# jonathanventura/spherical-sfm

Measured on AMD Instinct MI355X. Metric: BA obs/sec (Jac+Schur+PCG), higher is better.
Workload: dtype f64; 1 GPU; 300 cams x 100000 pts x 600000 obs synthetic circle (BASELINE configs[1]), general BA, focal fixed, CauchyLoss(1.0), Ceres-default LM; camera_dof=6, comm=none, reduced_solver=band-cholesky (direct), pcg_sweeps=0

## Files before the change

### spherical_sfm_amd/csrc/ba_kernels.h

```cpp
#pragma once
#include <hip/hip_runtime.h>
#include "ssfm_math.h"
#include "det_acc.h"

namespace ssfm {

static __global__ void k_profile_pad() {}

enum {
    SC_COST = 0,
    SC_FJJ = 1,
    SC_FJR = 2,
    SC_FWW = 3,
    SC_FWG = 4,
    SC_MODEL = 5,
    SC_STEP2_PT = 6,
    SC_XN2_PT = 7,
    SC_CAND_COST = 8,
    SC_X0N2_PT = 9,
    SC_NSUM = 10,
    SC_GMAX = 10,
    SC_STEP2_CAM = 11, SC_XN2_CAM = 12, SC_X0N2_CAM = 13,
    SC_TOTAL = 16
};
// ... 570 lines not shown
struct OctTR<N, 0> { static __device__ __forceinline__ void run(double (&v)[N], double* out) {
#pragma unroll
    for (int j = 0; j < N; j++) out[j] = v[j]; } };
__device__ __forceinline__ void wave_lds_handover() {
    __builtin_amdgcn_fence(__ATOMIC_RELEASE, "wavefront"); __builtin_amdgcn_wave_barrier(); __builtin_amdgcn_fence(__ATOMIC_ACQUIRE, "wavefront");
}
template <int DC> __device__ __forceinline__ constexpr bool jc_zero(int r, int i) { return DC == 6 && ((r == 0 && i == 1) || (r == 1 && i == 0)); }
__device__ __forceinline__ int gram_cam_of(int camv, int k) { return __shfl(camv, k, 64); }
template <int PER, int STRIDE, int NA>
__device__ __forceinline__ void gram_gather(const double* __restrict__ A, const double* __restrict__ B, int camv, int K, int lane, double* __restrict__ dst) {
    constexpr int NIT = (GRAM_KMAX * PER + 63) / 64;
    double v[NIT];
#pragma unroll
    for (int it = 0; it < NIT; it++) {
        const int e = lane + 64 * it, k = e / PER, i = e - PER * k;
        const int c = gram_cam_of(camv, min(k, K - 1));
        const double* src = (i < NA) ? A + 6 * (size_t)c + i : B + 27 * (size_t)c + (i - NA);
        v[it] = *src;
    }
#pragma unroll
    for (int it = 0; it < NIT; it++) {
        const int e = lane + 64 * it, k = e / PER, i = e - PER * k;
        if (e < K * PER) dst[k * STRIDE + i] = v[it];
    }
}
struct GramFuse { const double* scale_pt; double radius, min_diag, max_diag; double* PS_out; double* gp_out; double* scal; const double* spec; int emit_skip = 0; };
template <int DC, int NT, int TI, bool FUSE>
__device__ __forceinline__ void
schur_gram_task(const double* __restrict__ cam, const double* __restrict__ rot, const double* __restrict__ pts, const double* __restrict__ focal,
                const double2* __restrict__ obs_xy, const int* __restrict__ gr_rec, const double* __restrict__ scale_cam, const double* __restrict__ scale_f,
                const double* __restrict__ PS, int loss, double la, int rows_alloc, int focal_free, const int task, double* __restrict__ S_val, double* __restrict__ rhs,
                double* __restrict__ Udiag, double* __restrict__ Sfc, double* __restrict__ gcraw, long long* __restrict__ dbg, const GramFuse& fz, const DetZone& dz) {
    double fz_radius = fz.radius;
    if (FUSE && fz.spec) { if (fz.spec[0] == 0.0) return; fz_radius = fz.spec[1]; }
    constexpr int BB = DC * DC, off = (DC == 6) ? 0 : 3;
    constexpr int NU = DC * (DC + 1) / 2, NS = NU + 3 * DC, NO = (NS + 7) / 8;
    typedef double v4d_ __attribute__((ext_vector_type(4)));
    const long long t_0 = dbg ? wall_clock64() : 0;
    extern __shared__ __attribute__((aligned(16))) double sY[];
    const int lane = threadIdx.x & 63;
    double* sYw = sY + (size_t)(threadIdx.x >> 6) * (rows_alloc * GRAM_LD + GRAM_TAIL);
    double* sCam = sYw + rows_alloc * GRAM_LD;
    double* sScale = sCam + GRAM_KMAX * GRAM_CAMREC;
    int* sSlot = (int*)(sScale + 48);
    int* sDiag = sSlot + GRAM_NPAIR;
    const int* rec = gr_rec + (size_t)task * GRAM_REC;
    const int p0 = __builtin_amdgcn_readfirstlane(rec[0]), cnt = __builtin_amdgcn_readfirstlane(rec[1]), K = __builtin_amdgcn_readfirstlane(rec[2]);
    const int j00 = __builtin_amdgcn_readfirstlane(rec[3]);
    const double f = focal[0];
    const int camv = rec[4 + (lane & (GRAM_KMAX - 1))];
    gram_gather<33, GRAM_CAMREC, 6>(cam, rot, camv, K, lane, sCam);
    { const int k = min(lane / DC, K - 1), c = gram_cam_of(camv, k); const double sc = scale_cam[6 * c + off + lane - DC * (lane / DC)]; if (lane < DC * K) sScale[lane] = sc; }
    if (lane < GRAM_NPAIR + GRAM_KMAX) sSlot[lane] = rec[12 + lane];
    v4d_ acc[NT * (NT + 1) / 2];
#pragma unroll
    for (int t = 0; t < NT * (NT + 1) / 2; t++) acc[t] = v4d_{0.0, 0.0, 0.0, 0.0};
    double tacc[TI > 0 ? TI : 1] = {};
    double sm[NS];
#pragma unroll
    for (int i = 0; i < NS; i++) sm[i] = 0.0;
    const int li = lane & 15, lk = lane >> 4;
    const int lp = lane & (GRAM_SUB - 1), lq = lane >> 3;
    const int kq = min(lq, K - 1);
    const double sf = scale_f[0];
    double X[3], V[12]; double2 ob;
    double spt[3] = {0.0, 0.0, 0.0};
    double pacc[5] = {0.0, 0.0, 0.0, 0.0, 0.0}, pgmax = 0.0;
#define GRAM_LOAD(s0_)                                                                                                            \
    do {                                                                                                                          \
        const int q_ = min((s0_) + lp, cnt - 1);                                                                                  \
        _Pragma("unroll") for (int k = 0; k < 3; k++) X[k] = pts[3 * (size_t)(p0 + q_) + k];                                      \
        if (FUSE) { _Pragma("unroll") for (int k = 0; k < 3; k++) spt[k] = fz.scale_pt[3 * (size_t)(p0 + q_) + k]; }              \
        else {                                                                                                                    \
        _Pragma("unroll") for (int k = 0; k < 9; k++) V[k] = PS[12 * (size_t)(p0 + q_) + k];                                      \
        if (focal_free) { _Pragma("unroll") for (int k = 9; k < 12; k++) V[k] = PS[12 * (size_t)(p0 + q_) + k]; }                 \
        }                                                                                                                         \
        ob = obs_xy[j00 + (size_t)q_ * K + kq];                                                                                   \
    } while (0)
    GRAM_LOAD(0);
    long long t_1 = 0, t_2 = 0;
    for (int s0 = 0; s0 < cnt; s0 += GRAM_SUB) {
        wave_lds_handover();
        {
            const bool valid = s0 + lp < cnt;
            const double* crec = sCam + kq * GRAM_CAMREC;
            if (FUSE) {
                const double wgt = (valid && lq < K) ? 1.0 : 0.0;
                double pv[12];
                {
                    ObsPoint Lp; lin_obs_point(f, crec, crec + 6, X, ob.x, ob.y, loss, la, Lp);
                    double j0[2], j1[2], j2[2], jf[2];
#pragma unroll
                    for (int a = 0; a < 2; a++) { j0[a] = Lp.Jp[a][0] * spt[0] * wgt; j1[a] = Lp.Jp[a][1] * spt[1] * wgt; j2[a] = Lp.Jp[a][2] * spt[2] * wgt; jf[a] = Lp.Jf[a] * sf * wgt; }
                    pv[0] = j0[0] * j0[0] + j0[1] * j0[1]; pv[1] = j0[0] * j1[0] + j0[1] * j1[1]; pv[2] = j0[0] * j2[0] + j0[1] * j2[1];
                    pv[3] = j1[0] * j1[0] + j1[1] * j1[1]; pv[4] = j1[0] * j2[0] + j1[1] * j2[1]; pv[5] = j2[0] * j2[0] + j2[1] * j2[1];
                    pv[6] = j0[0] * Lp.r[0] + j0[1] * Lp.r[1]; pv[7] = j1[0] * Lp.r[0] + j1[1] * Lp.r[1]; pv[8] = j2[0] * Lp.r[0] + j2[1] * Lp.r[1];
                    pv[9] = jf[0] * j0[0] + jf[1] * j0[1]; pv[10] = jf[0] * j1[0] + jf[1] * j1[1]; pv[11] = jf[0] * j2[0] + jf[1] * j2[1];
                    pacc[0] += wgt * Lp.half_rho; pacc[1] += jf[0] * jf[0] + jf[1] * jf[1]; pacc[2] += jf[0] * Lp.r[0] + jf[1] * Lp.r[1];
                }
#pragma unroll
                for (int i = 0; i < 12; i++) { double t = pv[i]; t += __shfl_xor(t, 8, 64); t += __shfl_xor(t, 16, 64); t += __shfl_xor(t, 32, 64); pv[i] = t; }
                double Vd[6] = {pv[0], pv[1], pv[2], pv[3], pv[4], pv[5]};
                if (spt[0] > 0.0) {
                    if (valid && lq == 0) pgmax = fmax(pgmax, fmax(fabs(pv[6] / spt[0]), fmax(fabs(pv[7] / spt[1]), fabs(pv[8] / spt[2]))));
                    Vd[0] += fmin(fmax(Vd[0], fz.min_diag), fz.max_diag) / fz_radius;
                    Vd[3] += fmin(fmax(Vd[3], fz.min_diag), fz.max_diag) / fz_radius;
                    Vd[5] += fmin(fmax(Vd[5], fz.min_diag), fz.max_diag) / fz_radius;
                } else { Vd[0] = Vd[3] = Vd[5] = 1.0; }
                double Vi[6]; sym3_inverse(Vd, Vi);
                const double u0 = pv[9] * Vi[0] + pv[10] * Vi[1] + pv[11] * Vi[2];
                const double u1 = pv[9] * Vi[1] + pv[10] * Vi[3] + pv[11] * Vi[4];
                const double u2 = pv[9] * Vi[2] + pv[10] * Vi[4] + pv[11] * Vi[5];
                V[0] = Vi[0] * spt[0] * spt[0]; V[1] = Vi[1] * spt[0] * spt[1]; V[2] = Vi[2] * spt[0] * spt[2];
                V[3] = Vi[3] * spt[1] * spt[1]; V[4] = Vi[4] * spt[1] * spt[2]; V[5] = Vi[5] * spt[2] * spt[2];
                V[6] = spt[0] * (Vi[0] * pv[6] + Vi[1] * pv[7] + Vi[2] * pv[8]); V[7] = spt[1] * (Vi[1] * pv[6] + Vi[3] * pv[7] + Vi[4] * pv[8]);
                V[8] = spt[2] * (Vi[2] * pv[6] + Vi[4] * pv[7] + Vi[5] * pv[8]);
                V[9] = spt[0] * u0; V[10] = spt[1] * u1; V[11] = spt[2] * u2;
                if (valid && lq == 0) {
                    pacc[3] += u0 * pv[9] + u1 * pv[10] + u2 * pv[11];
                    pacc[4] += u0 * pv[6] + u1 * pv[7] + u2 * pv[8];
                    double* ps = fz.PS_out + 12 * (size_t)(p0 + s0 + lp);
#pragma unroll
                    for (int k = 0; k < 12; k++) ps[k] = V[k];
#pragma unroll
                    for (int k = 0; k < 3; k++) fz.gp_out[3 * (size_t)(p0 + s0 + lp) + k] = pv[6 + k];
                }
            }
            ObsLin Lk; lin_obs<DC == 6>(f, crec, crec + 6, X, ob.x, ob.y, loss, la, Lk);
            double L00 = 0, L10 = 0, L20 = 0, L11 = 0, L21 = 0, L22 = 0;
            if (valid && V[0] > 0.0) {
                const double i0 = fast_rsqrt(V[0]);
                L00 = V[0] * i0; L10 = V[1] * i0; L20 = V[2] * i0;
                const double d1 = V[3] - L10 * L10;
                if (d1 > 0.0) {
                    const double i1 = fast_rsqrt(d1);
                    L11 = d1 * i1; L21 = (V[4] - L20 * L10) * i1;
                    const double d2 = V[5] - L20 * L20 - L21 * L21;
                    if (d2 > 0.0) L22 = d2 * fast_rsqrt(d2);
                }
            }
            double Jc[2][DC]; cam_block_raw<DC>(Lk, Jc);
            double T[2][3];
#pragma unroll
            for (int r = 0; r < 2; r++) {
                T[r][0] = Lk.Jp[r][0] * L00 + Lk.Jp[r][1] * L10 + Lk.Jp[r][2] * L20;
                T[r][1] = Lk.Jp[r][1] * L11 + Lk.Jp[r][2] * L21;
                T[r][2] = Lk.Jp[r][2] * L22;
            }
            if (lq < K) {
                double* dst = sYw + (size_t)(DC * kq) * GRAM_LD + 3 * lp;
#pragma unroll
                for (int d = 0; d < DC; d++)
#pragma unroll
                    for (int cc = 0; cc < 3; cc++) {
                        double y = 0.0;
                        if (!jc_zero<DC>(0, d)) y += Jc[0][d] * T[0][cc];
                        if (!jc_zero<DC>(1, d)) y += Jc[1][d] * T[1][cc];
                        dst[d * GRAM_LD + cc] = y;
                    }
                if (valid) {
                    double yv[2], zv[2];
#pragma unroll
                    for (int r = 0; r < 2; r++) {
                        yv[r] = Lk.Jp[r][0] * V[6] + Lk.Jp[r][1] * V[7] + Lk.Jp[r][2] * V[8];
                        zv[r] = focal_free ? Lk.Jf[r] * sf - (Lk.Jp[r][0] * V[9] + Lk.Jp[r][1] * V[10] + Lk.Jp[r][2] * V[11]) : 0.0;
                    }
                    int u = 0;
#pragma unroll
                    for (int a2 = 0; a2 < DC; a2++) {
#pragma unroll
                        for (int b2 = a2; b2 < DC; b2++) {
                            if (!jc_zero<DC>(0, a2) && !jc_zero<DC>(0, b2)) sm[u] += Jc[0][a2] * Jc[0][b2];
                            if (!jc_zero<DC>(1, a2) && !jc_zero<DC>(1, b2)) sm[u] += Jc[1][a2] * Jc[1][b2];
                            u++;
                        }
#pragma unroll
                        for (int r = 0; r < 2; r++)
                            if (!jc_zero<DC>(r, a2)) {
                                sm[NU + a2] += Jc[r][a2] * Lk.r[r];
                                sm[NU + DC + a2] -= Jc[r][a2] * yv[r];
// ... 76 lines not shown
        if (lq < K) {
            const int c = cam_k;
            const double* sc = sScale + DC * lq;
            const int i0 = 4 * (lane & 1) + 2 * ((lane >> 1) & 1) + ((lane >> 2) & 1);
#pragma unroll
            for (int j = 0; j < NO; j++) {
                const int i = 8 * j + i0;
                const double v = out[j];
                if (i < NU) {
                    int a = 0, rem = i; while (rem >= DC - a) { rem -= DC - a; a++; }
                    const int b = a + rem;
                    const double w = v * sc[a] * sc[b];
                    sG[g_off(DC * lq + b) + DC * lq + a] += w;
                    if (b == a) { if (PV) PV[lq * 5 * DC + a] = w; else zadd(dz, &Udiag[c * DC + a], w); }
                } else if (i < NU + DC) { const int a = i - NU; if (PV) { PV[lq * 5 * DC + DC + a] = v * sc[a]; PV[lq * 5 * DC + 3 * DC + a] = v * sc[a]; } else { zadd(dz, &rhs[c * DC + a], v * sc[a]); zadd(dz, &gcraw[c * DC + a], v * sc[a]); } }
                else if (i < NU + 2 * DC) { const int a = i - NU - DC; if (PV) PV[lq * 5 * DC + 2 * DC + a] = v * sc[a]; else zadd(dz, &rhs[c * DC + a], v * sc[a]); }
                else if (i < NS && focal_free) { const int a = i - NU - 2 * DC; if (PV) PV[lq * 5 * DC + 4 * DC + a] = v * sc[a]; else zadd(dz, &Sfc[c * DC + a], v * sc[a]); }
            }
        }
    }
    wave_lds_handover();
    if constexpr (2 * BB > 64) {
        const int e = min(lane, BB - 1), da = e / DC, db = e - da * DC, eT = db * DC + da;
        const bool on = lane < BB;
        for (int a = 0; a < K; a++) {
            const int Ra = DC * a + da;
            for (int b = 0; b <= a; b++) {
                const int C = DC * b + db;
                const double v = sG[(b < a) ? g_off(Ra) + C : g_off(max(Ra, C)) + min(Ra, C)];
                const int sl = (b < a) ? sSlot[a * (a - 1) / 2 + b] : sDiag[a];
                const int eo = (b < a && (sl & (1 << 30))) ? eT : e;
                if (on) {
                    if (PB) PB[(a * (a + 1) / 2 + b) * BB + eo] = v;
                    else zadd(dz, &(S_val + (size_t)(sl & 0x3fffffff) * BB)[eo], v);
                }
            }
        }
    } else {
        const int nent = (K * (K + 1) / 2) * BB;
        for (int idx = lane; idx < nent; idx += 64) {
            const int blk = idx / BB, e = idx - blk * BB, da = e / DC, db = e - da * DC;
            const int a = (int)((__fsqrt_rn((float)(8 * blk + 1)) - 1.0f) * 0.5f);
            const int b = blk - a * (a + 1) / 2;
            const int R = DC * a + da, C = DC * b + db;
            const double v = sG[g_off(max(R, C)) + min(R, C)];
            if (b < a) {
                const int sl = sSlot[a * (a - 1) / 2 + b];
                const int eo = (sl & (1 << 30)) ? (db * DC + da) : e;
                if (PB) PB[blk * BB + eo] = v;
                else zadd(dz, &(S_val + (size_t)(sl & 0x3fffffff) * BB)[eo], v);
            } else if (PB) PB[idx] = v;
            else zadd(dz, &(S_val + (size_t)sDiag[a] * BB)[e], v);
        }
    }
    if (FUSE) {
        const double t = wave_transpose_sum(pacc);
        pgmax = wave_max(pgmax);
        const int slot = wave_tr_index();
        double* sl = fz.scal + (size_t)(task & (SC_NSLOT - 1)) * SC_TOTAL;
        if (slot < 5) unsafeAtomicAdd(&sl[slot], t);
        if (lane == 0 && pgmax > 0.0) atomic_max_nonneg(&sl[SC_GMAX], pgmax);
    }
    if (dbg && lane == 0) { long long* d = dbg + 4 * (size_t)task; d[0] = t_0; d[1] = t_1; d[2] = t_2; d[3] = wall_clock64(); }
}

template <int DC, int NT, int TI = 0, bool FUSE = false>
__global__ void __launch_bounds__(256) __attribute__((amdgpu_waves_per_eu(2)))
k_schur_gram(const double* __restrict__ cam, const double* __restrict__ rot, const double* __restrict__ pts, const double* __restrict__ focal,
             const double2* __restrict__ obs_xy, int ntasks, const int* __restrict__ gr_rec, const double* __restrict__ scale_cam, const double* __restrict__ scale_f,
             const double* __restrict__ PS, int loss, double la, int rows_alloc, int focal_free, int task0, double* __restrict__ S_val, double* __restrict__ rhs,
             double* __restrict__ Udiag, double* __restrict__ Sfc, double* __restrict__ gcraw, long long* __restrict__ dbg, GramFuse fz = GramFuse{}, DetZone dz = DetZone{}) {
    const int task = task0 + __builtin_amdgcn_readfirstlane(xcd_contiguous_block(blockIdx.x, gridDim.x) * (blockDim.x >> 6) + (threadIdx.x >> 6));
    if (task >= ntasks) return;
    schur_gram_task<DC, NT, TI, FUSE>(cam, rot, pts, focal, obs_xy, gr_rec, scale_cam, scale_f, PS, loss, la, rows_alloc, focal_free, task, S_val, rhs, Udiag, Sfc, gcraw, dbg, fz, dz);
}
template <int DC>
__global__ void __launch_bounds__(256) __attribute__((amdgpu_waves_per_eu(2)))
k_schur_gram_any(const double* __restrict__ cam, const double* __restrict__ rot, const double* __restrict__ pts, const double* __restrict__ focal,
                 const double2* __restrict__ obs_xy, int ntasks, const int* __restrict__ gr_rec, const double* __restrict__ scale_cam, const double* __restrict__ scale_f,
                 const double* __restrict__ PS, int loss, double la, int rows_alloc, int focal_free, int use_t4, double* __restrict__ S_val, double* __restrict__ rhs,
                 double* __restrict__ Udiag, double* __restrict__ Sfc, double* __restrict__ gcraw, DetZone dz = DetZone{}) {
    const int task = ntasks - 1 - __builtin_amdgcn_readfirstlane(xcd_contiguous_block(blockIdx.x, gridDim.x) * (blockDim.x >> 6) + (threadIdx.x >> 6));
    if (task < 0) return;
    const int rows = DC * __builtin_amdgcn_readfirstlane(gr_rec[(size_t)task * GRAM_REC + 2]);
    const GramFuse fz{};
#define SSFM_GRAM_ANY(NT_, TI_) schur_gram_task<DC, NT_, TI_, false>(cam, rot, pts, focal, obs_xy, gr_rec, scale_cam, scale_f, PS, loss, la, rows_alloc, focal_free, task, S_val, rhs, Udiag, Sfc, gcraw, nullptr, fz, dz)
    if (rows <= 16) SSFM_GRAM_ANY(1, 0);
    else if (rows <= 20 && use_t4) SSFM_GRAM_ANY(1, 2);
    else if (rows <= 32) SSFM_GRAM_ANY(2, 0);
    else if (DC == 6 && rows <= 36 && use_t4) SSFM_GRAM_ANY(2, 3);
    else if (DC == 6) SSFM_GRAM_ANY(3, 0);
#undef SSFM_GRAM_ANY
}

template <int DC>
__global__ void __launch_bounds__(256, 3)
k_pairs_y_probe(const int* __restrict__ row_ptr, const int* __restrict__ col_idx, const int* __restrict__ task_cam, const int* __restrict__ task_b0,
                const int* __restrict__ task_b1, int ntasks, const int* __restrict__ batch_slot, const int* __restrict__ pair_j,
                const int* __restrict__ pair_j2, const double* __restrict__ scale_cam, const double* __restrict__ Y, double* __restrict__ S_scratch) {
    constexpr int BB = DC * DC, YW = DC * 3;
    const int lane = threadIdx.x & 63;
    const int task = __builtin_amdgcn_readfirstlane(xcd_contiguous_block(blockIdx.x, gridDim.x) * (blockDim.x >> 6) + (threadIdx.x >> 6));
    if (task >= ntasks) return;
    const int c = __builtin_amdgcn_readfirstlane(task_cam[task]);
    const int b0 = __builtin_amdgcn_readfirstlane(task_b0[task]), b1 = __builtin_amdgcn_readfirstlane(task_b1[task]);
    const int rb = __builtin_amdgcn_readfirstlane(row_ptr[c]);
    double blk[DC][DC];
#pragma unroll
    for (int a = 0; a < DC; a++)
#pragma unroll
        for (int b = 0; b < DC; b++) blk[a][b] = 0.0;
    int cur = -1;
    const int tr_slot = wave_tr_index();
    auto fold = [&]() {
// ... 1017 lines not shown
```

### spherical_sfm_amd/csrc/ba_solver.hip

```cpp
#include <atomic>
#include <hip/hip_runtime.h>
#include <chrono>
#include <cmath>
#include <cstdlib>
#include <cstring>
#include <limits>
#include <string>
#include <vector>
#include "ba_flatten.h"
#include "ba_kernels.h"
#include "band_kernels.h"
#include "knobs.h"
#include "ssfm_ctx.h"

#include "ba_handle.h"

namespace ssfm {

constexpr unsigned DET_K_ASSEMBLY = (1u << SC_COST) | (1u << SC_FJJ) | (1u << SC_FJR) | (1u << SC_FWW) | (1u << SC_FWG);
constexpr unsigned DET_K_TAIL = (1u << SC_MODEL) | (1u << SC_STEP2_PT) | (1u << SC_XN2_PT) | (1u << SC_CAND_COST) | (1u << SC_STEP2_CAM) | (1u << SC_XN2_CAM);
static unsigned det_tail_mask(bool with_cams, bool gram_fold) {
    const unsigned tail = with_cams ? (DET_K_TAIL & ~((1u << SC_STEP2_CAM) | (1u << SC_XN2_CAM))) : DET_K_TAIL;
    return tail | (gram_fold ? (1u << SC_COST) : 0u);
}
// ... 32 lines not shown
    static int pl_block() { return SSFM_LAB_KNOB("SSFM_PL_BLOCK", 64); }
    static bool fused_publish() { return SSFM_LAB_KNOB("SSFM_PUBLISH_FUSED", 0) != 0; }
    static bool zone_clear_fused() { return SSFM_LAB_KNOB("SSFM_ZONE_CLEAR_FUSED", 1) != 0; }

    struct ZoneView { double *scal, *S_val, *rhs, *Udiag, *Sfc, *gcraw; DetZone det; const double* fold_part; long long* fold_lacc; };
    ZoneView zone(int iter) const {
        ZoneView z; z.scal = h->zone.p + (size_t)(iter & 1) * h->zone_len;
        z.S_val = z.scal + h->scal.n + h->pcg.n; z.rhs = z.S_val + h->zone_nnz; z.Udiag = z.rhs + (h->zone_n + 1); z.Sfc = z.Udiag + h->zone_n; z.gcraw = z.Sfc + h->zone_n;
        if (h->det) { z.det.base = z.S_val; z.det.limb = h->det_limb.p + 1; }
        if (h->gram_fold) { z.det.part = h->gram_part.p; z.det.part_off = h->gpart_off.p; }
        z.fold_part = h->gram_fold ? h->gram_part.p : (const double*)nullptr; z.fold_lacc = h->gram_fold ? lacc : (long long*)nullptr;
        return z;
    }
    struct NextClear { double* zone; double2* in_finalize; size_t len2; };
    NextClear next_clear() const {
        NextClear n; n.zone = zone(iteration + 1).scal;
        const bool fused = O.preconditioner == 0 && zone_clear_fused() && (h->zone_len % 2 == 0) && ((reinterpret_cast<uintptr_t>(n.zone) & 15) == 0);
        n.in_finalize = fused ? reinterpret_cast<double2*>(n.zone) : (double2*)nullptr; n.len2 = fused ? h->zone_len / 2 : 0;
        return n;
    }
    void det_decode(const ZoneView& z, bool matrices, unsigned kmask) {
        const int gz = matrices ? (int)std::min<size_t>(512, (h->det_nacc + 255) / 256) : 0;
        LAUNCH(h, KID_DET_DECODE, k_det_decode, gz + 1, 256, 0, z.S_val, h->det_limb.p + 1, h->det_nacc, gz, z.scal, h->det_lacc.p, kmask);
    }
    int record_phase(int i) { if (phases) SSFM_HIP_CHECK(ctx, hipEventRecord(h->phase_ev[i], st)); return SSFM_OK; }

    int wait_iteration() {
        if (!poll || h->profile || (h->opt.verbose != 0)) SSFM_HIP_CHECK(ctx, hipStreamSynchronize(st));
        const int rc = poll ? wait_published(h) : SSFM_OK; if (rc) return rc;
        if (!poll) {
            double* host_sp = h->host_sp;
            for (int k = 0; k < SC_TOTAL; k++) {
                double a = host_sp[k];
                for (int s2 = 1; s2 < SC_NSLOT; s2++) { const double v = host_sp[(size_t)s2 * SC_TOTAL + k]; a = (k == SC_GMAX) ? std::max(a, v) : a + v; }
                host_sp[k] = a;
            }
        }
        return SSFM_OK;
    }
    int need_x0() {
        if (!x0_pending) return SSFM_OK;
        SSFM_HIP_CHECK(ctx, hipEventSynchronize(h->x0_ev));
        x_norm = std::sqrt(host_scal[SC_X0N2_PT] + host_scal[SC_X0N2_CAM]); x0_pending = false;
        return SSFM_OK;
    }

    int read_knobs() {
        poll = lm_poll() && publish_alloc(h);
        if (!poll && !h->host_sp) SSFM_HIP_CHECK(ctx, hipHostMalloc((void**)&h->host_sp, (SC_NSLOT * SC_TOTAL + PCG_TOTAL + 1) * sizeof(double), hipHostMallocDefault));
        host_scal = poll ? h->host_pub : h->host_sp; host_pcg1 = poll ? h->host_pub + SC_TOTAL : h->host_sp + SC_NSLOT * SC_TOTAL;
        spec_on = poll && nP > 0 && knob_env_int("SSFM_LM_SPECULATE", 1) != 0;
        gram_bs = knob_env_int("SSFM_GRAM_BACKSUB", -1);
        gbs_split_env = knob_env_int("SSFM_GBS_SPLIT", 0);
        fuse_lin = SSFM_LAB_KNOB("SSFM_GRAM_FUSE", 0) != 0 && nP > 0 && !F.gr_rec.empty() && F.gram_points == (int64_t)nP && F.chunk_cam.empty() && F.cs_task_cam.empty();
        return SSFM_OK;
    }

    int startup() {
        { const int rc = read_knobs(); if (rc) return rc; }
        const int gp_pts = (nP + 255) / 256;
        h->set_zone(0);
        if (h->det) {
            if (!h->gram_fold) SSFM_HIP_CHECK(ctx, hipMemsetAsync(h->det_limb.p, 0, (2 * h->det_nacc + 2) * sizeof(long long), st));
            SSFM_HIP_CHECK(ctx, h->clear_det_lacc());
        }
        const bool make_scale = !h->scale_ready;
        LAUNCH(h, KID_CAM_ROT, k_cam_rot0, gp_cam, 64, 0, x.cam, x.rot, Nc, h->scal.p, (int)SC_TOTAL, h->diag_f.p, make_scale ? 1 : 0);
        if (make_scale) {
            if (nP > 0) hipLaunchKernelGGL(k_colnorm_both, dim3(gp_pts + Nc), dim3(256), 0, st, gp_pts, x.cam, x.rot, x.pts, x.focal, oxy, h->obs_cam.p, h->pt_start.p, nP,
                                           loss, la, h->diag_pt.p, h->diag_f.p, h->mask_pt.p, h->scale_pt.p, O.jacobi_scaling, h->det ? h->det_dfpart.p : (double*)nullptr,
                                           h->obs_pt.p, h->cam_start.p, h->cam_obs.p, h->diag_cam.p, h->mask_cam.p, ctx->collective ? (double*)nullptr : h->scale_cam.p);
            else hipLaunchKernelGGL(k_colnorm_cam, dim3(Nc), dim3(256), 0, st, x.cam, x.rot, x.pts, x.focal, oxy, h->obs_pt.p, h->cam_start.p, h->cam_obs.p,
                               loss, la, h->diag_cam.p, h->mask_cam.p, ctx->collective ? (double*)nullptr : h->scale_cam.p, O.jacobi_scaling);
            if (ctx->collective) {
                int rc = allreduce(h, h->diag_cam.p, (size_t)Nc * 6, ncclSum); if (rc) return rc;
                rc = allreduce(h, h->diag_f.p, 1, ncclSum); if (rc) return rc;
            }
            h->scale_ready = true;
        }
        {
            const int gpt = nP > 0 ? std::min(256, (nP * 3 + 255) / 256) : 0, gcm = std::min(16, (Nc * 6 + 255) / 256);
            hipLaunchKernelGGL(k_startup_tail, dim3(gpt + gcm), dim3(256), 0, st, x.pts, h->mask_pt.p, nP * 3, gpt, x.cam, h->mask_cam.p, Nc * 6, x.focal, h->mask_f.p,
                               h->diag_cam.p, (make_scale && ctx->collective) ? h->scale_cam.p : (double*)nullptr, h->diag_f.p, make_scale ? h->scale_f.p : (double*)nullptr,
                               O.jacobi_scaling, h->scal.p + SC_X0N2_PT, h->scal.p + SC_X0N2_CAM, (make_scale && h->det && nP > 0) ? h->det_dfpart.p : (const double*)nullptr, gp_pts,
                               (const double*)h->scal.p, lacc);
            if (h->det) LAUNCH(h, KID_DET_DECODE, k_det_decode, 1, 256, 0, h->S_val, h->det_limb.p + 1, h->det_nacc, 0, h->scal.p, h->det_lacc.p, (1u << SC_X0N2_PT) | (1u << SC_X0N2_CAM));
        }
        { int rc = allreduce(h, h->scal.p + SC_X0N2_PT, 1, ncclSum); if (rc) return rc; }
        SSFM_HIP_CHECK(ctx, hipMemcpyAsync(host_scal, h->scal.p, SC_TOTAL * sizeof(double), hipMemcpyDeviceToHost, st));
        if (!h->x0_ev) SSFM_HIP_CHECK(ctx, hipEventCreateWithFlags(&h->x0_ev, hipEventDisableTiming));
        SSFM_HIP_CHECK(ctx, hipEventRecord(h->x0_ev, st));
        SSFM_HIP_CHECK(ctx, hipMemsetAsync(zone(1).scal, 0, h->zone_len * sizeof(double), st));
        S->num_successful_steps = 1; S->num_unsuccessful_steps = 0; S->num_linearizations = 0; S->pcg_iterations_total = 0;
        S->termination = SSFM_NO_CONVERGENCE;
        if (fused_publish() && poll && !h->pub_ticket.p) {
            SSFM_HIP_CHECK(ctx, h->pub_ticket.alloc(1)); SSFM_HIP_CHECK(ctx, hipMemsetAsync(h->pub_ticket.p, 0, sizeof(int), st));
        }
        if (phases) for (auto& e : h->phase_ev) if (!e) SSFM_HIP_CHECK(ctx, hipEventCreate(&e));
#ifdef SSFM_LAB
        { const int rc = lab_y_probe_alloc(); if (rc) return rc; }
#endif
        return SSFM_OK;
    }

    void point_lin(const State& at, double* scal, const double* spec) {
        const int PLB = pl_block();
        LAUNCH(h, KID_POINT_LIN, k_point_lin<3>, (nP + PLB - 1) / PLB, PLB, 0, at.cam, at.rot, at.pts, at.focal, oxy, h->obs_cam.p, h->pt_start.p, nP, h->scale_pt.p,
               h->scale_f.p, loss, la, radius, O.min_lm_diagonal, O.max_lm_diagonal, h->Vs.p, h->gp.p, scal, spec, lacc);
    }
    void finalize_gather(const ZoneView& z, const NextClear& nc) {
        const bool merged = F.band_block != DC;
        const auto kernel = merged ? (h->gram_fold ? k_finalize_gather<DC, true, true> : k_finalize_gather<DC, true, false>)
                                   : (h->gram_fold ? k_finalize_gather<DC, false, true> : k_finalize_gather<DC, false, false>);
        LAUNCH(h, KID_FINALIZE, kernel, Nc, 256, 0, h->row_ptr.p, h->col_idx.p, h->diag_slot.p, h->scale_cam.p, h->scale_f.p, z.Udiag, z.gcraw,
               radius, O.min_lm_diagonal, O.max_lm_diagonal, Nc, h->cam_pos.p, h->cam_pos2.p, h->pair_dummy.p, F.y_rows(DC), F.band, z.S_val, z.rhs, z.Sfc, h->Sff.p, h->band.p, h->Yb.p,
               z.scal, nc.in_finalize, nc.len2, h->col_pos.p, h->wrap_ptr_p(), h->wrap_blk.p, h->wrap_row2.p,
               z.fold_part, (const int*)nullptr, h->fold_slot_src.p, z.Udiag, z.gcraw, z.Sfc, z.fold_lacc);
        h->band_filled = true;
    }
    void point_backsub(int lpp, bool res, const unsigned char* skip, const LmGate* fused, double* spec) {
        const int PTB = pt_block();
        const auto kernel = lpp != 2 ? k_point_backsub<DC, 1> : k_point_backsub<DC, 2>;
        LAUNCH(h, KID_BACKSUB, kernel, (lpp * nP + PTB - 1) / PTB + (res ? 1 : 0), PTB, 0, x.cam, x.rot, x.pts, x.focal, oxy, h->obs_cam.p, h->pt_start.p, nP, h->scale_cam.p,
               h->scale_pt.p, h->scale_f.p, h->Vs.p, h->gp.p, h->px.p, Nc, loss, la, c.cam, c.rot, c.focal, c.pts, h->scal.p,
               h->rhs, h->pq.p, h->Sfc, h->Sff.p, O.pcg_tolerance * O.pcg_tolerance, res ? h->pr.p : (double*)nullptr, h->pcg.p, skip,
               fused ? h->pub_ticket.p : (int*)nullptr, fused ? h->host_pub : (double*)nullptr, fused ? ++ctx->pub_seq : 0ull, fused ? *fused : LmGate(), spec,
               fused ? (long long*)nullptr : lacc);
    }
    void gram_backsub(bool res) {
        const int ng = (int)(F.gr_rec.size() / GRAM_REC);
        const int gbs_wave_target = 14 * ctx->num_cus;
        const int gbs_split = gbs_split_env > 0 ? std::min(8, gbs_split_env) : std::max(1, std::min(4, (gbs_wave_target + ng - 1) / std::max(1, ng)));
        LAUNCH(h, KID_GRAM_BACKSUB, k_gram_backsub2<DC>, (ng * gbs_split + GBS_WAVES - 1) / GBS_WAVES + (res ? 1 : 0), 64 * GBS_WAVES, GBS_WAVES * GBS2_TAIL * sizeof(double), x.cam, x.rot, x.pts, x.focal, oxy, ng, h->gr_rec.p,
               h->scale_cam.p, h->scale_f.p, h->Vs.p, h->px.p, Nc, loss, la, c.cam, c.rot, c.focal, c.pts, h->scal.p,
               h->rhs, h->pq.p, h->Sfc, h->Sff.p, O.pcg_tolerance * O.pcg_tolerance, res ? h->pr.p : (double*)nullptr, h->pcg.p, lacc, gbs_split);
    }
    using GramKernel = decltype(&k_schur_gram<DC, 1, 0, false>);
    template <bool FUSE> static GramKernel gram_kernel_of(int cls) {
        static const GramKernel k[5] = {k_schur_gram<DC, 1, 0, FUSE>, k_schur_gram<DC, 1, 2, FUSE>, k_schur_gram<DC, 2, 0, FUSE>, k_schur_gram<DC, 2, 3, FUSE>, k_schur_gram<DC, 3, 0, FUSE>};
        return k[cls];
    }
    GramKernel gram_kernel(int cls) const {
#ifdef SSFM_LAB
        if (fuse_lin) return gram_kernel_of<true>(cls);
#endif
        return gram_kernel_of<false>(cls);
    }
    int launch_gram(const State& at, const ZoneView& z, const double* spec) {
        const int ng = (int)(F.gr_rec.size() / GRAM_REC);
        const bool gram_t4 = SSFM_LAB_KNOB("SSFM_GRAM_T4", 1) != 0;
        const int gram_waves = std::min(4, std::max(1, SSFM_LAB_KNOB("SSFM_GRAM_WAVES", 1)));
        long long* gram_dbg = nullptr;
#ifdef SSFM_LAB
        gram_dbg = lab_gram_stamps_begin(ng);
#endif
        auto tile_class = [&](int K) { const int rows = DC * K; return rows <= 16 ? 0 : (rows <= 20 && gram_t4) ? 1 : rows <= 32 ? 2 : (rows <= 36 && gram_t4) ? 3 : 4; };
        int cls_end[5] = {0, 0, 0, 0, 0};
        for (int t = 0; t < ng; t++) { const int c0 = tile_class(F.gr_rec[(size_t)t * GRAM_REC + 2]); for (int cl = c0; cl < 5; cl++) cls_end[cl] = t + 1; }
        int n_cls = 0; for (int cl = 0; cl < 5; cl++) if (cls_end[cl] > (cl ? cls_end[cl - 1] : 0)) n_cls++;
        const bool gram_any = F.gram_any;
        bool any_ok = gram_any && n_cls > 1 && gram_waves == 1 && !gram_dbg;
#ifdef SSFM_LAB
        any_ok = any_ok && !fuse_lin;
#endif
        if (any_ok) {
            const int rows_alloc = DC * F.gr_rec[(size_t)(ng - 1) * GRAM_REC + 2];
            const size_t gram_lds = ((size_t)rows_alloc * GRAM_LD + GRAM_TAIL) * sizeof(double);
            if (gram_lds > 48 * 1024) SSFM_HIP_CHECK(ctx, hipFuncSetAttribute(reinterpret_cast<const void*>(k_schur_gram_any<DC>), hipFuncAttributeMaxDynamicSharedMemorySize, (int)gram_lds));
            LAUNCH(h, KID_SCHUR_GRAM, (k_schur_gram_any<DC>), ng, 64, gram_lds, at.cam, at.rot, at.pts, at.focal, oxy, ng, h->gr_rec.p, h->scale_cam.p, h->scale_f.p, h->Vs.p, loss, la, rows_alloc,
                   F.focal_free ? 1 : 0, gram_t4 ? 1 : 0, z.S_val, z.rhs, z.Udiag, z.Sfc, z.gcraw, z.det);
        } else {
            GramFuse fz; fz.scale_pt = h->scale_pt.p; fz.radius = radius; fz.min_diag = O.min_lm_diagonal; fz.max_diag = O.max_lm_diagonal; fz.PS_out = h->Vs.p; fz.gp_out = h->gp.p; fz.scal = z.scal; fz.emit_skip = SSFM_LAB_KNOB("SSFM_GRAM_EMIT_SKIP", 0); fz.spec = spec;
            for (int cl = 0; cl < (DC == 6 ? 5 : 3); cl++) {
                const int t0 = cl ? cls_end[cl - 1] : 0, t1 = cls_end[cl];
                if (t1 <= t0) continue;
                const GramKernel kernel = gram_kernel(cl);
                const int rows_alloc = DC * F.gr_rec[(size_t)(t1 - 1) * GRAM_REC + 2];
                const size_t gram_lds = (size_t)gram_waves * ((size_t)rows_alloc * GRAM_LD + GRAM_TAIL) * sizeof(double);
                if (gram_lds > 48 * 1024) SSFM_HIP_CHECK(ctx, hipFuncSetAttribute(reinterpret_cast<const void*>(kernel), hipFuncAttributeMaxDynamicSharedMemorySize, (int)gram_lds));
                LAUNCH(h, KID_SCHUR_GRAM, kernel, (t1 - t0 + gram_waves - 1) / gram_waves, 64 * gram_waves, gram_lds, at.cam, at.rot, at.pts, at.focal, oxy, t1, h->gr_rec.p,
                       h->scale_cam.p, h->scale_f.p, h->Vs.p, loss, la, rows_alloc, F.focal_free ? 1 : 0, t0, z.S_val, z.rhs, z.Udiag, z.Sfc, z.gcraw, gram_dbg, fz, z.det);
            }
        }
#ifdef SSFM_LAB
        if (gram_dbg) lab_gram_stamps_print(gram_dbg, ng);
#endif
        return SSFM_OK;
    }

    int assemble() {
        h->set_zone(iteration & 1);
        const ZoneView z = zone(iteration);
        { const int rc = record_phase(0); if (rc) return rc; }
        if (h->profile && nP > 0 && !lin_done) hipLaunchKernelGGL(k_profile_pad, dim3(1), dim3(64), 0, st);
        if (nP > 0 && !lin_done && !fuse_lin) point_lin(x, z.scal, nullptr);
        { const int rc = record_phase(1); if (rc) return rc; }
        if (!F.cs_task_cam.empty()) {
            const int ntasks = (int)F.cs_task_cam.size();
            LAUNCH(h, KID_CAM_SUMS, k_cam_sums2<DC>, (ntasks + 3) / 4, 256, 0, x.cam, x.rot, x.pts, x.focal, oxy, h->cam_obs.p, h->cam_obs_pt.p, h->cs_task_cam.p,
                   h->cs_task_q0.p, h->cs_task_q1.p, ntasks, h->row_ptr.p, h->diag_slot.p, h->scale_cam.p, h->scale_f.p, h->Vs.p, loss, la, z.S_val, z.rhs,
                   z.Udiag, z.Sfc, z.gcraw, (const unsigned char*)(F.gram_points > 0 ? h->pt_grouped.p : nullptr), z.det);
        }
        if (!F.chunk_cam.empty()) {
            const int ntasks = (int)F.chunk_cam.size();
            auto kernel = k_schur_pairs2<DC>; bool occ3 = false;
#ifdef SSFM_LAB
            occ3 = SSFM_LAB_KNOB("SSFM_PAIRS_OCC3", 0) != 0 && DC == 6;
            if (occ3) kernel = k_schur_pairs2<DC, 3>;
#endif
            LAUNCH(h, KID_SCHUR_ROWS, kernel, (ntasks + 3) / 4, 256, 0, x.cam, x.rot, x.pts, x.focal, oxy, h->row_ptr.p, h->col_idx.p, h->chunk_cam.p,
                   h->chunk_b0.p, h->chunk_b1.p, ntasks, h->batch_slot.p, h->pair_j.p, h->pair_j2.p, h->pair_p.p, h->scale_cam.p, h->Vs.p, loss, la, z.S_val,
                   occ3 ? DetZone{} : z.det);
        }
        if (!F.gr_rec.empty() && !(fuse_lin && lin_done)) {
            const int rc = launch_gram(x, z, nullptr); if (rc) return rc;
        }
        lin_done = false;
#ifdef SSFM_LAB
        lab_y_probe_launch();
#endif
        if (h->det && !h->gram_fold) {
            det_decode(z, true, DET_K_ASSEMBLY);
            SSFM_HIP_CHECK(ctx, hipMemsetAsync(h->det_limb.p, 0, sizeof(long long), st));
// ... 784 lines not shown
```

Before: 3.546 billion obs/s.

## Enable fused point-block linearization in gram kernel with per-point prologue

Restructures the fused path of the Schur gram kernel. Each lane now linearizes all observations of one point in a prologue, builds and inverts the 3x3 point block, writes PS and gp, and reduces the scalars before the main gram loop. The old version computed per observation and reduced with cross-lane shuffles inside the tiled loop. The fused path is also enabled by default (no longer lab-only) when there is no det mode, no mixed-class any-kernel, and no class-4 tiles, which removes a separate point-linearization pass. The cost is a serial loop over K per lane and a global write and re-read of PS within the kernel.

```diff
diff --git a/spherical_sfm_amd/csrc/ba_kernels.h b/spherical_sfm_amd/csrc/ba_kernels.h
--- a/spherical_sfm_amd/csrc/ba_kernels.h
+++ b/spherical_sfm_amd/csrc/ba_kernels.h
@@ -646,6 +646,74 @@
     gram_gather<33, GRAM_CAMREC, 6>(cam, rot, camv, K, lane, sCam);
     { const int k = min(lane / DC, K - 1), c = gram_cam_of(camv, k); const double sc = scale_cam[6 * c + off + lane - DC * (lane / DC)]; if (lane < DC * K) sScale[lane] = sc; }
     if (lane < GRAM_NPAIR + GRAM_KMAX) sSlot[lane] = rec[12 + lane];
+    const double sf = scale_f[0];
+    if constexpr (FUSE) {
+        double pacc[5] = {0.0, 0.0, 0.0, 0.0, 0.0}, pgmax = 0.0;
+        constexpr int KC = ((16 * NT + (TI > 0 ? 4 : 0)) / DC < GRAM_KMAX) ? (16 * NT + (TI > 0 ? 4 : 0)) / DC : GRAM_KMAX;
+        wave_lds_handover();
+        for (int r0 = 0; r0 < cnt; r0 += 64) {
+            const bool valid = r0 + lane < cnt;
+            const int q = min(r0 + lane, cnt - 1);
+            const size_t p = (size_t)(p0 + q);
+            const double2* op = obs_xy + (j00 + (size_t)q * K);
+            double Xp[3], sp[3]; double2 oo[KC];
+#pragma unroll
+            for (int k = 0; k < 3; k++) { Xp[k] = pts[3 * p + k]; sp[k] = fz.scale_pt[3 * p + k]; }
+#pragma unroll
+            for (int k = 0; k < KC; k++) oo[k] = op[min(k, K - 1)];
+            double Vd[6] = {0, 0, 0, 0, 0, 0}, g[3] = {0, 0, 0}, wf[3] = {0, 0, 0}, a0 = 0.0, a1 = 0.0, a2 = 0.0;
+#pragma unroll
+            for (int k = 0; k < KC; k++)
+                if (k < K) {
+                    const double* crec = sCam + k * GRAM_CAMREC;
+                    ObsPoint L; lin_obs_point(f, crec, crec + 6, Xp, oo[k].x, oo[k].y, loss, la, L);
+                    a0 += L.half_rho;
+#pragma unroll
+                    for (int a = 0; a < 2; a++) {
+                        const double j0 = L.Jp[a][0] * sp[0], j1 = L.Jp[a][1] * sp[1], j2 = L.Jp[a][2] * sp[2], jf = L.Jf[a] * sf;
+                        Vd[0] += j0 * j0; Vd[1] += j0 * j1; Vd[2] += j0 * j2; Vd[3] += j1 * j1; Vd[4] += j1 * j2; Vd[5] += j2 * j2;
+                        g[0] += j0 * L.r[a]; g[1] += j1 * L.r[a]; g[2] += j2 * L.r[a];
+                        wf[0] += jf * j0; wf[1] += jf * j1; wf[2] += jf * j2;
+                        a1 += jf * jf; a2 += jf * L.r[a];
+                    }
+                }
+            double gm = 0.0;
+            if (sp[0] > 0.0) {
+                gm = fmax(fabs(g[0] / sp[0]), fmax(fabs(g[1] / sp[1]), fabs(g[2] / sp[2])));
+                Vd[0] += fmin(fmax(Vd[0], fz.min_diag), fz.max_diag) / fz_radius;
+                Vd[3] += fmin(fmax(Vd[3], fz.min_diag), fz.max_diag) / fz_radius;
+                Vd[5] += fmin(fmax(Vd[5], fz.min_diag), fz.max_diag) / fz_radius;
+            } else { Vd[0] = Vd[3] = Vd[5] = 1.0; }
+            double Vi[6]; sym3_inverse(Vd, Vi);
+            const double u0 = wf[0] * Vi[0] + wf[1] * Vi[1] + wf[2] * Vi[2];
+            const double u1 = wf[0] * Vi[1] + wf[1] * Vi[3] + wf[2] * Vi[4];
+            const double u2 = wf[0] * Vi[2] + wf[1] * Vi[4] + wf[2] * Vi[5];
+            if (valid) {
+                pacc[0] += a0; pacc[1] += a1; pacc[2] += a2;
+                pacc[3] += u0 * wf[0] + u1 * wf[1] + u2 * wf[2];
+                pacc[4] += u0 * g[0] + u1 * g[1] + u2 * g[2];
+                pgmax = fmax(pgmax, gm);
+                double* ps = fz.PS_out + 12 * p;
+                ps[0] = Vi[0] * sp[0] * sp[0]; ps[1] = Vi[1] * sp[0] * sp[1]; ps[2] = Vi[2] * sp[0] * sp[2];
+                ps[3] = Vi[3] * sp[1] * sp[1]; ps[4] = Vi[4] * sp[1] * sp[2]; ps[5] = Vi[5] * sp[2] * sp[2];
+                ps[6] = sp[0] * (Vi[0] * g[0] + Vi[1] * g[1] + Vi[2] * g[2]); ps[7] = sp[1] * (Vi[1] * g[0] + Vi[3] * g[1] + Vi[4] * g[2]);
+                ps[8] = sp[2] * (Vi[2] * g[0] + Vi[4] * g[1] + Vi[5] * g[2]);
+                ps[9] = sp[0] * u0; ps[10] = sp[1] * u1; ps[11] = sp[2] * u2;
+#pragma unroll
+                for (int k = 0; k < 3; k++) fz.gp_out[3 * p + k] = g[k];
+            }
+        }
+        {
+            const double t = wave_transpose_sum(pacc);
+            pgmax = wave_max(pgmax);
+            const int slot = wave_tr_index();
+            double* sl = fz.scal + (size_t)(task & (SC_NSLOT - 1)) * SC_TOTAL;
+            if (slot < 5) unsafeAtomicAdd(&sl[slot], t);
+            if (lane == 0 && pgmax > 0.0) atomic_max_nonneg(&sl[SC_GMAX], pgmax);
+        }
+        __builtin_amdgcn_fence(__ATOMIC_RELEASE, "workgroup"); __builtin_amdgcn_s_waitcnt(0x0F70 ); __builtin_amdgcn_fence(__ATOMIC_ACQUIRE, "workgroup");
+    }
+    const double* PSr = FUSE ? (const double*)fz.PS_out : PS;
     v4d_ acc[NT * (NT + 1) / 2];
 #pragma unroll
     for (int t = 0; t < NT * (NT + 1) / 2; t++) acc[t] = v4d_{0.0, 0.0, 0.0, 0.0};
@@ -656,19 +724,13 @@
     const int li = lane & 15, lk = lane >> 4;
     const int lp = lane & (GRAM_SUB - 1), lq = lane >> 3;
     const int kq = min(lq, K - 1);
-    const double sf = scale_f[0];
     double X[3], V[12]; double2 ob;
-    double spt[3] = {0.0, 0.0, 0.0};
-    double pacc[5] = {0.0, 0.0, 0.0, 0.0, 0.0}, pgmax = 0.0;
 #define GRAM_LOAD(s0_)                                                                                                            \
     do {                                                                                                                          \
         const int q_ = min((s0_) + lp, cnt - 1);                                                                                  \
         _Pragma("unroll") for (int k = 0; k < 3; k++) X[k] = pts[3 * (size_t)(p0 + q_) + k];                                      \
-        if (FUSE) { _Pragma("unroll") for (int k = 0; k < 3; k++) spt[k] = fz.scale_pt[3 * (size_t)(p0 + q_) + k]; }              \
-        else {                                                                                                                    \
-        _Pragma("unroll") for (int k = 0; k < 9; k++) V[k] = PS[12 * (size_t)(p0 + q_) + k];                                      \
-        if (focal_free) { _Pragma("unroll") for (int k = 9; k < 12; k++) V[k] = PS[12 * (size_t)(p0 + q_) + k]; }                 \
-        }                                                                                                                         \
+        _Pragma("unroll") for (int k = 0; k < 9; k++) V[k] = PSr[12 * (size_t)(p0 + q_) + k];                                     \
+        if (focal_free) { _Pragma("unroll") for (int k = 9; k < 12; k++) V[k] = PSr[12 * (size_t)(p0 + q_) + k]; }                \
         ob = obs_xy[j00 + (size_t)q_ * K + kq];                                                                                   \
     } while (0)
     GRAM_LOAD(0);
@@ -678,48 +740,6 @@
         {
             const bool valid = s0 + lp < cnt;
             const double* crec = sCam + kq * GRAM_CAMREC;
-            if (FUSE) {
-                const double wgt = (valid && lq < K) ? 1.0 : 0.0;
-                double pv[12];
-                {
-                    ObsPoint Lp; lin_obs_point(f, crec, crec + 6, X, ob.x, ob.y, loss, la, Lp);
-                    double j0[2], j1[2], j2[2], jf[2];
-#pragma unroll
-                    for (int a = 0; a < 2; a++) { j0[a] = Lp.Jp[a][0] * spt[0] * wgt; j1[a] = Lp.Jp[a][1] * spt[1] * wgt; j2[a] = Lp.Jp[a][2] * spt[2] * wgt; jf[a] = Lp.Jf[a] * sf * wgt; }
-                    pv[0] = j0[0] * j0[0] + j0[1] * j0[1]; pv[1] = j0[0] * j1[0] + j0[1] * j1[1]; pv[2] = j0[0] * j2[0] + j0[1] * j2[1];
-                    pv[3] = j1[0] * j1[0] + j1[1] * j1[1]; pv[4] = j1[0] * j2[0] + j1[1] * j2[1]; pv[5] = j2[0] * j2[0] + j2[1] * j2[1];
-                    pv[6] = j0[0] * Lp.r[0] + j0[1] * Lp.r[1]; pv[7] = j1[0] * Lp.r[0] + j1[1] * Lp.r[1]; pv[8] = j2[0] * Lp.r[0] + j2[1] * Lp.r[1];
-                    pv[9] = jf[0] * j0[0] + jf[1] * j0[1]; pv[10] = jf[0] * j1[0] + jf[1] * j1[1]; pv[11] = jf[0] * j2[0] + jf[1] * j2[1];
-                    pacc[0] += wgt * Lp.half_rho; pacc[1] += jf[0] * jf[0] + jf[1] * jf[1]; pacc[2] += jf[0] * Lp.r[0] + jf[1] * Lp.r[1];
-                }
-#pragma unroll
-                for (int i = 0; i < 12; i++) { double t = pv[i]; t += __shfl_xor(t, 8, 64); t += __shfl_xor(t, 16, 64); t += __shfl_xor(t, 32, 64); pv[i] = t; }
-                double Vd[6] = {pv[0], pv[1], pv[2], pv[3], pv[4], pv[5]};
-                if (spt[0] > 0.0) {
-                    if (valid && lq == 0) pgmax = fmax(pgmax, fmax(fabs(pv[6] / spt[0]), fmax(fabs(pv[7] / spt[1]), fabs(pv[8] / spt[2]))));
-                    Vd[0] += fmin(fmax(Vd[0], fz.min_diag), fz.max_diag) / fz_radius;
-                    Vd[3] += fmin(fmax(Vd[3], fz.min_diag), fz.max_diag) / fz_radius;
-                    Vd[5] += fmin(fmax(Vd[5], fz.min_diag), fz.max_diag) / fz_radius;
-                } else { Vd[0] = Vd[3] = Vd[5] = 1.0; }
-                double Vi[6]; sym3_inverse(Vd, Vi);
-                const double u0 = pv[9] * Vi[0] + pv[10] * Vi[1] + pv[11] * Vi[2];
-                const double u1 = pv[9] * Vi[1] + pv[10] * Vi[3] + pv[11] * Vi[4];
-                const double u2 = pv[9] * Vi[2] + pv[10] * Vi[4] + pv[11] * Vi[5];
-                V[0] = Vi[0] * spt[0] * spt[0]; V[1] = Vi[1] * spt[0] * spt[1]; V[2] = Vi[2] * spt[0] * spt[2];
-                V[3] = Vi[3] * spt[1] * spt[1]; V[4] = Vi[4] * spt[1] * spt[2]; V[5] = Vi[5] * spt[2] * spt[2];
-                V[6] = spt[0] * (Vi[0] * pv[6] + Vi[1] * pv[7] + Vi[2] * pv[8]); V[7] = spt[1] * (Vi[1] * pv[6] + Vi[3] * pv[7] + Vi[4] * pv[8]);
-                V[8] = spt[2] * (Vi[2] * pv[6] + Vi[4] * pv[7] + Vi[5] * pv[8]);
-                V[9] = spt[0] * u0; V[10] = spt[1] * u1; V[11] = spt[2] * u2;
-                if (valid && lq == 0) {
-                    pacc[3] += u0 * pv[9] + u1 * pv[10] + u2 * pv[11];
-                    pacc[4] += u0 * pv[6] + u1 * pv[7] + u2 * pv[8];
-                    double* ps = fz.PS_out + 12 * (size_t)(p0 + s0 + lp);
-#pragma unroll
-                    for (int k = 0; k < 12; k++) ps[k] = V[k];
-#pragma unroll
-                    for (int k = 0; k < 3; k++) fz.gp_out[3 * (size_t)(p0 + s0 + lp) + k] = pv[6 + k];
-                }
-            }
             ObsLin Lk; lin_obs<DC == 6>(f, crec, crec + 6, X, ob.x, ob.y, loss, la, Lk);
             double L00 = 0, L10 = 0, L20 = 0, L11 = 0, L21 = 0, L22 = 0;
             if (valid && V[0] > 0.0) {
@@ -902,14 +922,6 @@
             } else if (PB) PB[idx] = v;
             else zadd(dz, &(S_val + (size_t)sDiag[a] * BB)[e], v);
         }
-    }
-    if (FUSE) {
-        const double t = wave_transpose_sum(pacc);
-        pgmax = wave_max(pgmax);
-        const int slot = wave_tr_index();
-        double* sl = fz.scal + (size_t)(task & (SC_NSLOT - 1)) * SC_TOTAL;
-        if (slot < 5) unsafeAtomicAdd(&sl[slot], t);
-        if (lane == 0 && pgmax > 0.0) atomic_max_nonneg(&sl[SC_GMAX], pgmax);
     }
     if (dbg && lane == 0) { long long* d = dbg + 4 * (size_t)task; d[0] = t_0; d[1] = t_1; d[2] = t_2; d[3] = wall_clock64(); }
 }
diff --git a/spherical_sfm_amd/csrc/ba_solver.hip b/spherical_sfm_amd/csrc/ba_solver.hip
--- a/spherical_sfm_amd/csrc/ba_solver.hip
+++ b/spherical_sfm_amd/csrc/ba_solver.hip
@@ -108,7 +108,9 @@
         spec_on = poll && nP > 0 && knob_env_int("SSFM_LM_SPECULATE", 1) != 0;
         gram_bs = knob_env_int("SSFM_GRAM_BACKSUB", -1);
         gbs_split_env = knob_env_int("SSFM_GBS_SPLIT", 0);
-        fuse_lin = SSFM_LAB_KNOB("SSFM_GRAM_FUSE", 0) != 0 && nP > 0 && !F.gr_rec.empty() && F.gram_points == (int64_t)nP && F.chunk_cam.empty() && F.cs_task_cam.empty();
+        { int cls_end[5]; const int n_cls = gram_classes(cls_end);
+          fuse_lin = knob_env_int("SSFM_GRAM_FUSE", 1) != 0 && !h->det && nP > 0 && !F.gr_rec.empty() && F.gram_points == (int64_t)nP && F.chunk_cam.empty() && F.cs_task_cam.empty()
+                     && !(F.gram_any && n_cls > 1) && cls_end[4] == cls_end[3]; }
         return SSFM_OK;
     }
 
@@ -193,38 +195,36 @@
     }
     using GramKernel = decltype(&k_schur_gram<DC, 1, 0, false>);
     template <bool FUSE> static GramKernel gram_kernel_of(int cls) {
-        static const GramKernel k[5] = {k_schur_gram<DC, 1, 0, FUSE>, k_schur_gram<DC, 1, 2, FUSE>, k_schur_gram<DC, 2, 0, FUSE>, k_schur_gram<DC, 2, 3, FUSE>, k_schur_gram<DC, 3, 0, FUSE>};
+        static const GramKernel k[5] = {k_schur_gram<DC, 1, 0, FUSE>, k_schur_gram<DC, 1, 2, FUSE>, k_schur_gram<DC, 2, 0, FUSE>, k_schur_gram<DC, 2, 3, FUSE && DC == 6>, k_schur_gram<DC, 3, 0, false>};
         return k[cls];
     }
-    GramKernel gram_kernel(int cls) const {
-#ifdef SSFM_LAB
-        if (fuse_lin) return gram_kernel_of<true>(cls);
-#endif
-        return gram_kernel_of<false>(cls);
+    GramKernel gram_kernel(int cls) const { return fuse_lin ? gram_kernel_of<true>(cls) : gram_kernel_of<false>(cls); }
+    static bool gram_t4() { return SSFM_LAB_KNOB("SSFM_GRAM_T4", 1) != 0; }
+    int gram_classes(int (&cls_end)[5]) const {
+        const int ng = (int)(F.gr_rec.size() / GRAM_REC);
+        const bool t4 = gram_t4();
+        auto tile_class = [&](int K) { const int rows = DC * K; return rows <= 16 ? 0 : (rows <= 20 && t4) ? 1 : rows <= 32 ? 2 : (rows <= 36 && t4) ? 3 : 4; };
+        for (int cl = 0; cl < 5; cl++) cls_end[cl] = 0;
+        for (int t = 0; t < ng; t++) { const int c0 = tile_class(F.gr_rec[(size_t)t * GRAM_REC + 2]); for (int cl = c0; cl < 5; cl++) cls_end[cl] = t + 1; }
+        int n_cls = 0; for (int cl = 0; cl < 5; cl++) if (cls_end[cl] > (cl ? cls_end[cl - 1] : 0)) n_cls++;
+        return n_cls;
     }
     int launch_gram(const State& at, const ZoneView& z, const double* spec) {
         const int ng = (int)(F.gr_rec.size() / GRAM_REC);
-        const bool gram_t4 = SSFM_LAB_KNOB("SSFM_GRAM_T4", 1) != 0;
         const int gram_waves = std::min(4, std::max(1, SSFM_LAB_KNOB("SSFM_GRAM_WAVES", 1)));
         long long* gram_dbg = nullptr;
 #ifdef SSFM_LAB
         gram_dbg = lab_gram_stamps_begin(ng);
 #endif
-        auto tile_class = [&](int K) { const int rows = DC * K; return rows <= 16 ? 0 : (rows <= 20 && gram_t4) ? 1 : rows <= 32 ? 2 : (rows <= 36 && gram_t4) ? 3 : 4; };
-        int cls_end[5] = {0, 0, 0, 0, 0};
-        for (int t = 0; t < ng; t++) { const int c0 = tile_class(F.gr_rec[(size_t)t * GRAM_REC + 2]); for (int cl = c0; cl < 5; cl++) cls_end[cl] = t + 1; }
-        int n_cls = 0; for (int cl = 0; cl < 5; cl++) if (cls_end[cl] > (cl ? cls_end[cl - 1] : 0)) n_cls++;
+        int cls_end[5]; const int n_cls = gram_classes(cls_end);
         const bool gram_any = F.gram_any;
-        bool any_ok = gram_any && n_cls > 1 && gram_waves == 1 && !gram_dbg;
-#ifdef SSFM_LAB
-        any_ok = any_ok && !fuse_lin;
-#endif
+        const bool any_ok = gram_any && n_cls > 1 && gram_waves == 1 && !gram_dbg && !fuse_lin;
         if (any_ok) {
             const int rows_alloc = DC * F.gr_rec[(size_t)(ng - 1) * GRAM_REC + 2];
             const size_t gram_lds = ((size_t)rows_alloc * GRAM_LD + GRAM_TAIL) * sizeof(double);
             if (gram_lds > 48 * 1024) SSFM_HIP_CHECK(ctx, hipFuncSetAttribute(reinterpret_cast<const void*>(k_schur_gram_any<DC>), hipFuncAttributeMaxDynamicSharedMemorySize, (int)gram_lds));
             LAUNCH(h, KID_SCHUR_GRAM, (k_schur_gram_any<DC>), ng, 64, gram_lds, at.cam, at.rot, at.pts, at.focal, oxy, ng, h->gr_rec.p, h->scale_cam.p, h->scale_f.p, h->Vs.p, loss, la, rows_alloc,
-                   F.focal_free ? 1 : 0, gram_t4 ? 1 : 0, z.S_val, z.rhs, z.Udiag, z.Sfc, z.gcraw, z.det);
+                   F.focal_free ? 1 : 0, gram_t4() ? 1 : 0, z.S_val, z.rhs, z.Udiag, z.Sfc, z.gcraw, z.det);
         } else {
             GramFuse fz; fz.scale_pt = h->scale_pt.p; fz.radius = radius; fz.min_diag = O.min_lm_diagonal; fz.max_diag = O.max_lm_diagonal; fz.PS_out = h->Vs.p; fz.gp_out = h->gp.p; fz.scal = z.scal; fz.emit_skip = SSFM_LAB_KNOB("SSFM_GRAM_EMIT_SKIP", 0); fz.spec = spec;
             for (int cl = 0; cl < (DC == 6 ? 5 : 3); cl++) {
```

Measured after the change: 3.691 billion obs/s, median of 6. 4.1% higher.
